# Kotstantinovskiy/SonicDiffusionBayesLab

Hardware: AMD Instinct MI355X
Metric: 512x512 images/sec at 50 DDIM steps (higher is better)
Workload: dtype bf16; 1 GPU; SD-1.5 512x512 DDIM 50 steps, CFG 7.5, batch=8/GPU (BASELINE configs[1]); global_batch=8, sample_size=64, parallelism=batch-shard x1, weights=SD-1.5-shaped synthetic seed 1234

## Files before the change

include/sd_hip.h:

```cpp
#ifndef SD_HIP_H
#define SD_HIP_H

#ifdef __cplusplus
extern "C" {
#endif

typedef struct sd_unet sd_unet;

typedef struct sd_unet_config {
    int sample_size;
    int in_channels;
    int out_channels;
    int num_levels;
    int block_out_channels[8];
    int layers_per_block;
    int attn_levels[8];
    int cross_attention_dim;
    int num_heads;
    int norm_num_groups;
    float norm_eps;
    int context_len;
    int weight_dtype;
    float fp8_act_scale_norm;
    float fp8_act_scale_ff;
// ... 123 lines not shown
                   int Cin, int Cout);
int sd_op_time_embedding(void* stream, float t, const void* W1, const float* b1, const void* W2, const float* b2,
                         float* scratch, float* temb, int dim_in, int dim);
int sd_op_timestep_cond(void* stream, float t, const float* cond, const void* Wc, float* row, float* emb, int cond_dim,
                        int dim);

int sd_op_ln_partials(int kind, int M, int N);
int sd_op_gemm_rowstats(void* stream, const void* X, long long ldx, const void* W, const float* bias, const void* R,
                        long long ldr, void* C, long long ldc, int M, int N, int K, float* rowstats);
int sd_op_gemm_ln(void* stream, const void* X, long long ldx, const void* Wg, const float* c1, const float* c2,
                  const float* rowstats, int parts, float eps, void* C, long long ldc, int M, int N, int K, int epi);
int sd_op_gemm_plan(void* stream, const void* X, long long ldx, const void* X2, long long ldx2, int K1, const void* W,
                    const float* bias, const float* bias2, const void* R, long long ldr, void* C, long long ldc, int M, int N,
                    int K, float* rowstats, float* stats, const float* ln_rs, int ln_parts, const float* ln_c1, float ln_eps,
                    void* KV, int hm_tokens);
int sd_op_xattn_fused_rowstats(void* stream, const void* X, const void* R, void* Y, const void* At, const void* Bw,
                               const float* bias, int M, int C, int rows_per_sample, int L, float* rowstats);
int sd_op_xattn_fused(void* stream, const void* X, const void* R, void* Y, const void* At, const void* Bw,
                      const float* bias, int M, int C, int rows_per_sample, int L);
int sd_op_xattn_fused_ln(void* stream, const void* X, const void* R, void* Y, const void* At, const void* Bw,
                         const float* bias, int M, int C, int rows_per_sample, int L, const float* ln_rowstats, int ln_parts,
                         long long ln_rows, const float* c2, float eps, float* rowstats);
int sd_op_conv3x3_ablate(void* stream, const void* X, const void* W, void* Y, int B, int Hin, int Win, int Cin, int Cout,
                         int ablate);
int sd_op_xattn_fused_stamps(void* stream, const void* X, const void* R, void* Y, const void* At, const void* Bw,
                             const float* bias, int M, int C, int rows_per_sample, int L, unsigned long long* stamps);

int sd_op_gemm_fp8(void* stream, const void* X, long long ldx, const void* W, const float* wscale, float xscale,
                   const float* bias, const void* R, long long ldr, void* C, long long ldc, int M, int N, int K, int epi,
                   int out_fp8, float oscale);
// ... 14 lines not shown
```

sonicdiffusionbayeslab_amd/_lib.py:

```python
from __future__ import annotations

import ctypes as C
import os
import re
from typing import Optional

HERE = os.path.dirname(os.path.abspath(__file__))
LIB_PATH = os.environ.get("SD_AMD_LIB", os.path.join(HERE, "lib", "libsdhip.so"))
HEADER_PATH = os.path.normpath(os.path.join(HERE, "..", "include", "sd_hip.h"))

ABLATE_LIB_PATH = os.path.join(HERE, "lib", "libsdhip_ablate.so")

_lib: Optional[C.CDLL] = None
_ablate: Optional[C.CDLL] = None


class SdUnetConfig(C.Structure):
    _fields_ = [
        ("sample_size", C.c_int), ("in_channels", C.c_int), ("out_channels", C.c_int),
        ("num_levels", C.c_int), ("block_out_channels", C.c_int * 8), ("layers_per_block", C.c_int),
        ("attn_levels", C.c_int * 8), ("cross_attention_dim", C.c_int), ("num_heads", C.c_int),
        ("norm_num_groups", C.c_int), ("norm_eps", C.c_float), ("context_len", C.c_int),
        ("weight_dtype", C.c_int), ("fp8_act_scale_norm", C.c_float), ("fp8_act_scale_ff", C.c_float),
        ("time_cond_proj_dim", C.c_int),
# ... 68 lines not shown
    "sd_op_conv3x3_kernel": (_i, [_i, _i, _i, _i, _i, _i, _i, _i]),
    "sd_op_softmax_rows": (_i, [_vp, _vp, _ll, _i, _f]),
    "sd_op_layernorm": (_i, [_vp, _vp, _vp, _vp, _vp, _i, _i, _f]),
    "sd_op_attention": (_i, [_vp, _vp, _ll, _vp, _ll, _vp, _ll, _vp, _ll, _i, _i, _i, _i, _i, _f]),
    "sd_op_gemm_qkv_headmajor": (_i, [_vp, _vp, _ll, _vp, _vp, _vp, _i, _i, _i, _i]),
    "sd_op_attention_headmajor": (_i, [_vp, _vp, _ll, _vp, _vp, _vp, _ll, _i, _i, _i, _i, _i, _f]),
    "sd_op_clip_attention": (_i, [_vp, _vp, _vp, _i, _i, _i, _i]),
    "sd_op_conv_in": (_i, [_vp, _vp, _i, _vp, _vp, _vp, _i, _i, _i, _i, _i]),
    "sd_op_conv_out": (_i, [_vp, _vp, _vp, _vp, _vp, _i, _i, _i, _i, _i]),
    "sd_op_time_embedding": (_i, [_vp, _f, _vp, _vp, _vp, _vp, _vp, _vp, _i, _i]),
    "sd_op_timestep_cond": (_i, [_vp, _f, _vp, _vp, _vp, _vp, _i, _i]),
    "sd_op_ln_partials": (_i, [_i, _i, _i]),
    "sd_op_gemm_rowstats": (_i, [_vp, _vp, _ll, _vp, _vp, _vp, _ll, _vp, _ll, _i, _i, _i, _vp]),
    "sd_op_gemm_plan": (_i, [_vp, _vp, _ll, _vp, _ll, _i, _vp, _vp, _vp, _vp, _ll, _vp, _ll, _i, _i, _i, _vp, _vp, _vp, _i, _vp, _f,
                            _vp, _i]),
    "sd_op_gemm_ln": (_i, [_vp, _vp, _ll, _vp, _vp, _vp, _vp, _i, _f, _vp, _ll, _i, _i, _i, _i]),
    "sd_op_xattn_fused_rowstats": (_i, [_vp, _vp, _vp, _vp, _vp, _vp, _vp, _i, _i, _i, _i, _vp]),
    "sd_op_xattn_fused": (_i, [_vp, _vp, _vp, _vp, _vp, _vp, _vp, _i, _i, _i, _i]),
    "sd_op_xattn_fused_ln": (_i, [_vp, _vp, _vp, _vp, _vp, _vp, _vp, _i, _i, _i, _i, _vp, _i, _ll, _vp, _f, _vp]),
    "sd_op_xattn_fused_stamps": (_i, [_vp, _vp, _vp, _vp, _vp, _vp, _vp, _i, _i, _i, _i, _vp]),
    "sd_op_gemm_fp8": (_i, [_vp, _vp, _ll, _vp, _vp, _f, _vp, _vp, _ll, _vp, _ll, _i, _i, _i, _i, _i, _f]),
    "sd_op_conv3x3_fp8": (_i, [_vp, _vp, _vp, _vp, _f, _vp, _vp, _vp, _vp, _i, _i, _i, _i, _i, _i, _i]),
    "sd_op_groupnorm_fp8": (_i, [_vp, _vp, _i, _vp, _i, _vp, _vp, _vp, _i, _i, _i, _f, _i, _i, _f]),
    "sd_op_layernorm_fp8": (_i, [_vp, _vp, _vp, _vp, _vp, _i, _i, _i, _f, _f]),
    "sd_op_quantize_fp8": (_i, [_vp, _vp, _vp, _ll, _i, _i, _f]),
}


def load() -> C.CDLL:
    global _lib
# ... 44 lines not shown
```

sonicdiffusionbayeslab_amd/csrc/gemm_conv.hip:

```cpp
#include "common.h"
#include "kernels.h"

#include <stdlib.h>

#ifdef SD_ABLATE
#define SD_TUNE(p) ((p).tune)
#else
#define SD_TUNE(p) 0
#endif

namespace {

constexpr int AMODE_GEMM = 0;
constexpr int AMODE_CONV = 1;
constexpr int EPI_STD = 0;
constexpr int EPI_GEGLU = 1;
constexpr int EPI_SOFTMAX = 2;

constexpr int kPersistentGrid = 512;

template <int N>
__device__ __forceinline__ void wait_vmcnt() {
    asm volatile("s_waitcnt vmcnt(%0)" ::"n"(N) : "memory");
}
// ... 629 lines not shown

int sd_gemm_splitk(int M, int N, int K, int rows) {
    static const char* env = getenv("SD_SPLITK");
    if (env) return atoi(env) > 1 ? atoi(env) : 1;
    if (rows == 0) rows = sd_gemm_tile_rows(M, N, K);
    const int tiles = ((M + rows - 1) / rows) * ((N + 159) / 160);
    const int KT = K / 64;
    if (tiles >= 448) return 1;
    int want = (512 + tiles - 1) / tiles;
    int maxs = KT / 12;
    int s = want < maxs ? want : maxs;
    if (s > 8) s = 8;
    return s < 1 ? 1 : s;
}

static int check_fp8(const GemmArgs& a, const char* what) {
    SD_REQUIRE(a.wscale != nullptr && a.xscale_inv > 0.f, "%s fp8: weight scales / activation scale missing", what);
    SD_REQUIRE(a.K % 128 == 0 && a.K >= 128, "%s fp8: K=%d must be a positive multiple of 128", what, a.K);
    SD_REQUIRE(a.X2 == nullptr && a.K1 == a.K, "%s fp8: no second K segment", what);
    SD_REQUIRE(a.rows_per_batch == 0, "%s fp8: per-sample weights are bf16 only", what);
    SD_REQUIRE(((uintptr_t)a.X & 15) == 0 && ((uintptr_t)a.W & 15) == 0, "%s fp8: operands must be 16-byte aligned", what);
    return 0;
}

static int check_stats(const GemmArgs& a, int epi) {
    if (!a.stats) return 0;
    SD_REQUIRE(epi == EPI_STD && a.M % 64 == 0 && !(a.splitk > 1 && a.slab) && !a.out_fp8,
               "producer statistics: plain epilogue, M %% 64 == 0 and no split-K (M=%d splitk=%d)", a.M, a.splitk);
    return 0;
}
// ... 41 lines not shown
        SD_REQUIRE(a.N % 32 == 0, "geglu gemm: N=%d must be a multiple of 32", a.N);
        if (!lean_off && big_tile_mode() == 0 && sd_gemm_lean_applicable(a, 1)) return sd_launch_gemm_lean(a, 1, 256, stream);
        if (big_tile_ok(a.M, a.N, 128)) return launch<256, 128, 4, 2, 3, AMODE_GEMM, EPI_GEGLU>(a, stream);
        if (big_tile_mode() != 3 && a.N % 256 == 0) return launch<256, 256, 4, 2, 2, AMODE_GEMM, EPI_GEGLU>(a, stream);
        return launch<128, 128, 2, 2, 2, AMODE_GEMM, EPI_GEGLU>(a, stream);
    }
    SD_REQUIRE(a.rows_per_batch == 0 || a.rows_per_batch % 128 == 0,
               "gemm: rows_per_batch=%d must be a multiple of the 128-row tile", a.rows_per_batch);
    if (epi == EPI_SOFTMAX) {
        SD_REQUIRE(a.N % 80 == 0 && a.sm_valid > 0 && a.sm_valid <= 80 && a.R == nullptr && (a.bias == nullptr || a.ln_rs),
                   "softmax gemm: N=%d must be a multiple of 80, 0 < sm_valid=%d <= 80, no bias/residual", a.N, a.sm_valid);
        SD_REQUIRE(!a.ln_per_sample || (a.ln_rs && a.rows_per_batch > 0), "gemm: per-sample LayerNorm vectors need per-sample weights");
        return launch<128, 160, 2, 2, 2, AMODE_GEMM, EPI_SOFTMAX>(a, stream);
    }
    if (a.rows_per_batch) return launch<128, 160, 2, 2, 2, AMODE_GEMM, EPI_STD>(a, stream);
    if (!lean_off && big_tile_mode() == 0 && sd_gemm_lean_applicable(a, epi)) {
        const int rows = (!a.stats && !a.ln_rs && !a.hm_C) ? sd_gemm_tile_rows(a.M, a.N, a.K) : 128;
        return sd_launch_gemm_lean(a, 0, rows, stream);
    }
    if (big_tile_ok(a.M, a.N, 160)) return launch<256, 160, 4, 2, 3, AMODE_GEMM, EPI_STD>(a, stream);
    if (big_tile_mode() == 2) return launch<256, 160, 4, 2, 2, AMODE_GEMM, EPI_STD>(a, stream);
    if (!a.stats && !a.ln_rs && sd_gemm_tile_rows(a.M, a.N, a.K) == 64) return launch<64, 160, 2, 2, 2, AMODE_GEMM, EPI_STD>(a, stream);
    return launch<128, 160, 2, 2, 2, AMODE_GEMM, EPI_STD>(a, stream);
}

int sd_launch_conv3x3(const GemmArgs& a, hipStream_t stream) {
    if (check_stats(a, EPI_STD)) return -1;
    if (a.dt == 1) {
        if (check_fp8(a, "conv3x3")) return -1;
        SD_REQUIRE(a.Cin % 128 == 0, "conv3x3 fp8: Cin=%d must be a multiple of 128 (pad the channels)", a.Cin);
// ... 30 lines not shown
```

sonicdiffusionbayeslab_amd/csrc/gemm_lean.hip:

```cpp
#include "common.h"
#include "kernels.h"
#include <mutex>
#include <stdlib.h>

namespace {

typedef __amdgpu_buffer_rsrc_t rsrc_t;

struct LeanArgs {
    const void* X; const void* X2; const void* W; const void* R; void* C; void* KV;
    const float* vec0; const float* vec1;
    const float* ln_rs; float* rowstats; float* stats;
    unsigned x_bytes, x2_bytes, w_bytes, r_bytes, c_bytes, kv_bytes;
    int M, N, K, K1;
    int ldxb, ldx2b, ldwb, ldrb, ldcb;
    int tiles_m, tiles_n;
    float ln_eps, inv_k;
    int hm_tpc;
    int hm_tok_shift, hm_heads, hm_samples;
};

template <int N>
__device__ __forceinline__ void wait_vmcnt() {
    asm volatile("s_waitcnt vmcnt(%0)" ::"n"(N) : "memory");
}

__device__ __forceinline__ rsrc_t make_rsrc(const void* p, unsigned bytes) {
    return __builtin_amdgcn_make_buffer_rsrc((void*)p, 0, (int)bytes, 0x00020000);
}
__device__ __forceinline__ void dma16(rsrc_t r, void* lds_wave_base, int voff, int soff) {
    __builtin_amdgcn_raw_ptr_buffer_load_lds(r, LDS_PTR(lds_wave_base), 16, voff, soff, 0, 0);
}

template <int BM, int BN, int WAVES_M, int WAVES_N, int NP, bool GEGLU>
__global__ __launch_bounds__(WAVES_M* WAVES_N * 64, 2) void gemm_lean_kernel(const LeanArgs p) {
    constexpr bool LN = NP > 0;
    constexpr int NW = WAVES_M * WAVES_N;
    constexpr int WTM = BM / WAVES_M, WTN = BN / WAVES_N;
    constexpr int TM = WTM / 16, TN = WTN / 16;
    constexpr int XI = BM / 8, WI = BN / 8;
    static_assert(XI % NW == 0 && WI % NW == 0, "pieces split evenly over the waves");
    constexpr int XPW = XI / NW, WPW = WI / NW;
    constexpr int STAGE_BYTES = (BM + BN) * 128;
    static_assert(GEGLU ? TN % 4 == 0 : TN % 2 == 1, "store schedule: GEGLU pairs of output tiles; std TN / 2 paired + one 8-byte store");
    constexpr bool FRAG_DB = TM * TN * 4 + (TM + TN) * 8 <= 200;
    constexpr int TNH = GEGLU ? TN / 2 : TN;

    extern __shared__ __attribute__((aligned(16))) char smem[];
    char* lnbuf = smem + 2 * STAGE_BYTES;
    char* vecs = lnbuf + NW * 512;

    const int tid = threadIdx.x, lane = tid & 63;
    const int wave = __builtin_amdgcn_readfirstlane(tid >> 6);
    const int wm = wave % WAVES_M, wn = wave / WAVES_M;
    const int lrow = lane & 15, lq = lane >> 4;

    const int nblk = gridDim.x;
    int work;
    {
        const int q = nblk >> 3, r = nblk & 7, xcd = blockIdx.x & 7, idx = blockIdx.x >> 3;
        work = (xcd < r ? xcd * (q + 1) : r * (q + 1) + (xcd - r) * q) + idx;
    }
    const int nwork = p.tiles_m * p.tiles_n;
    if (work >= nwork) return;
// ... 18 lines not shown
        const int hl = (cl * 205) >> 13;
        vH[j] = ((hl << p.hm_tok_shift) + rowl) * 80 + (cl - hl * 40) * 2;
    }
    const int vLn = (wm * WTM + lane) * 8;
    const int vRs = rowl * 8;
    const int vSt = (wn * WTN + lq * 4) * 8;
    const int vVec = (wn * WTN + lane * 4) * 4;

    const int swz[2] = {((lq) ^ (lane & 7)) << 4, ((4 + lq) ^ (lane & 7)) << 4};
    const int xoff = (wm * WTM + lrow) * 128;
    const int woff = BM * 128 + (wn * WTN + lrow) * 128;

    const int KT = p.K >> 6;
    int m0 = tile_m * BM, n0 = tile_n * BN;

    auto stage = [&](int kt, int buf) {
        char* xs = smem + buf * STAGE_BYTES;
        char* ws = xs + BM * 128;
        const int k0 = kt * 64;
        if (LN || k0 < p.K1) {
            const int so = (m0 + wave * 8) * p.ldxb + k0 * 2;
#pragma unroll
            for (int i = 0; i < XPW; ++i) dma16(rX, xs + (wave + i * NW) * 1024, vX, so + i * (NW * 8) * p.ldxb);
        } else {
            const int so = (m0 + wave * 8) * p.ldx2b + (k0 - p.K1) * 2;
#pragma unroll
            for (int i = 0; i < XPW; ++i) dma16(rX2, xs + (wave + i * NW) * 1024, vX2, so + i * (NW * 8) * p.ldx2b);
        }
        const int sw = (n0 + wave * 8) * p.ldwb + k0 * 2;
#pragma unroll
// ... 7 lines not shown
        for (int t = 0; t < TM; ++t) xf[t] = *(const bf16x8*)(sb + xoff + t * 2048 + swz[ks]);
#pragma unroll
        for (int t = 0; t < TN; ++t) wf[t] = *(const bf16x8*)(sb + woff + t * 2048 + swz[ks]);
    };
    auto mfmas = [&](const bf16x8* xf, const bf16x8* wf) {
#pragma unroll
        for (int a = 0; a < TN; ++a)
#pragma unroll
            for (int b = 0; b < TM; ++b)
                acc[a][b] = __builtin_amdgcn_mfma_f32_16x16x32_bf16(wf[a], xf[b], acc[a][b], 0, 0, 0);
    };

    constexpr int EPI_STORES = GEGLU ? (TN / 4) * TM : (TN / 2 + 1) * TM;
    int g = 0;
    bool stores_pending = false;
    stage(0, 0);
    while (true) {
#pragma unroll
        for (int a = 0; a < TN; ++a)
#pragma unroll
            for (int b = 0; b < TM; ++b) acc[a][b] = f32x4{0.f, 0.f, 0.f, 0.f};
        for (int kt = 0; kt < KT - 1; ++kt) {
            if (kt == 0 && stores_pending) wait_vmcnt<EPI_STORES>();
            else wait_vmcnt<0>();
            __builtin_amdgcn_s_barrier();
            asm volatile("" ::: "memory");
            const char* sb = smem + ((g + kt) & 1) * STAGE_BYTES;
            load_frags(sb, 0, xf0, wf0);
            __builtin_amdgcn_sched_barrier(0);
            stage(kt + 1, (g + kt + 1) & 1);
            if (kt == 0 && wm == 0 && lane < WTN / 4) {
                glds16((const char*)p.vec0 + (long)n0 * 4 + (unsigned)vVec, vecs + wn * WTN * 4);
                glds16((const char*)p.vec1 + (long)n0 * 4 + (unsigned)vVec, vecs + BN * 4 + wn * WTN * 4);
            }
            __builtin_amdgcn_sched_barrier(0);
            if (FRAG_DB) {
                load_frags(sb, 1, xf1, wf1);
                mfmas(xf0, wf0);
                mfmas(xf1, wf1);
            } else {
                mfmas(xf0, wf0);
                load_frags(sb, 1, xf0, wf0);
                mfmas(xf0, wf0);
            }
        }
        wait_vmcnt<0>();
        __builtin_amdgcn_s_barrier();
        asm volatile("" ::: "memory");
        static_assert(!LN || WTM == 64, "LayerNorm fold: lane l owns row l of its wave's 64 rows");
        u32x2 ep[LN ? NP : (GEGLU ? 1 : TN * TM)];
        {
            const char* sb = smem + ((g + KT - 1) & 1) * STAGE_BYTES;
            load_frags(sb, 0, xf0, wf0);
            if (FRAG_DB) load_frags(sb, 1, xf1, wf1);
            if (LN) {
                const char* src = (const char*)p.ln_rs + (long)m0 * 8;
#pragma unroll
                for (int i = 0; i < NP; ++i) ep[i] = *(const u32x2*)((src + (long)i * p.M * 8) + (unsigned)vLn);
            } else if (!GEGLU && p.R) {
                const int so = m0 * p.ldrb + n0 * 2;
#pragma unroll
                for (int b = 0; b < TM; ++b)
#pragma unroll
                    for (int a = 0; a < TN; ++a)
                        ep[a * TM + b] = __builtin_bit_cast(u32x2, __builtin_amdgcn_raw_buffer_load_b64(rR, vR + a * 32, so + b * 16 * p.ldrb, 0));
            }
            __builtin_amdgcn_sched_barrier(0);
// ... 55 lines not shown
                for (int a = 0; a < TNH; ++a) {
                    const f32x4 bv = v0[a] + v1[a];
#pragma unroll
                    for (int b = 0; b < TM; ++b) acc[a0 + a][b] += bv;
                }
            }
        }

        const int em0 = m0, en0 = n0, etile_n = tile_n;
        work += nblk;
        const bool more = work < nwork;
        if (more) {
            tile_n += dn; tile_m += dm;
            if (tile_n >= p.tiles_n) { tile_n -= p.tiles_n; tile_m += 1; }
            m0 = tile_m * BM; n0 = tile_n * BN;
            stage(0, g & 1);
            stores_pending = true;
        }

        if (!LN && !GEGLU && WTM == 64 && p.stats) {
            char* dst = (char*)p.stats + ((long)((em0 + wm * WTM) >> 6) * p.N + en0) * 8 + (unsigned)vSt;
#pragma unroll
            for (int a = 0; a < TN; ++a) {
                float sv[4] = {0.f, 0.f, 0.f, 0.f}, qv[4] = {0.f, 0.f, 0.f, 0.f};
#pragma unroll
                for (int b = 0; b < TM; ++b) {
                    const unsigned p0 = pack2bf(acc[a][b][0], acc[a][b][1]), p1 = pack2bf(acc[a][b][2], acc[a][b][3]);
                    const float v[4] = {bflo(p0), bfhi(p0), bflo(p1), bfhi(p1)};
#pragma unroll
                    for (int j = 0; j < 4; ++j) { sv[j] += v[j]; qv[j] = __builtin_fmaf(v[j], v[j], qv[j]); }
                }
// ... 93 lines not shown
    if (hipGetDevice(&dev) != hipSuccess || dev < 0 || dev >= 16) return nullptr;
    std::lock_guard<std::mutex> lock(mu);
    if (!z[dev]) {
        float* p = nullptr;
        float probe = 1.f;
        if (hipMalloc((void**)&p, 16384 * 4) != hipSuccess) return nullptr;
        if (hipMemset(p, 0, 16384 * 4) != hipSuccess || hipMemcpy(&probe, p + 16383, 4, hipMemcpyDeviceToHost) != hipSuccess || probe != 0.f) {
            (void)hipFree(p);
            return nullptr;
        }
        z[dev] = p;
    }
    return z[dev];
}

template <int BM, int BN, int WAVES_M, int WAVES_N, int NP, bool GEGLU>
int launch_lean(const LeanArgs& a0, hipStream_t stream) {
    LeanArgs a = a0;
    a.tiles_m = (a.M + BM - 1) / BM;
    a.tiles_n = a.N / BN;
    constexpr int NW = WAVES_M * WAVES_N;
    constexpr int smem = 2 * (BM + BN) * 128 + NW * 512 + 2 * BN * 4;
    static_assert(smem <= 160 * 1024, "tile does not fit the 160 KiB LDS");
    auto kern = gemm_lean_kernel<BM, BN, WAVES_M, WAVES_N, NP, GEGLU>;
    static bool attr_set = false;
    if (!attr_set) {
        SD_CHECK_HIP(hipFuncSetAttribute((const void*)kern, hipFuncAttributeMaxDynamicSharedMemorySize, smem));
        attr_set = true;
    }
    int grid = a.tiles_m * a.tiles_n;
    constexpr int resident = smem > 80 * 1024 ? 256 : 512;
    if (grid > resident) grid = resident;
    hipLaunchKernelGGL(kern, dim3(grid), dim3(NW * 64), smem, stream, a);
    SD_CHECK_HIP(hipGetLastError());
    return 0;
}

}

// ... 10 lines not shown
    if (a.R && (long)a.M * a.ldr * 2 >= big) return false;
    if ((a.stats || a.rowstats || a.ln_rs || a.hm_C) && a.M % (epi ? 256 : 128) != 0) return false;
    if (a.ln_rs) {
        if (a.R || a.bias2 || !a.bias || !a.ln_c1 || a.X2 || a.K1 != a.K || a.stats || a.rowstats) return false;
        if (a.ln_np != 2 && a.ln_np != 4 && a.ln_np != 8 && a.ln_np != 16) return false;
    }
    if (epi == 1 && (a.R || a.bias2 || a.X2 || a.K1 != a.K || a.stats || a.rowstats || a.hm_C)) return false;
    if (a.hm_C) {
        if (!a.ln_rs || !a.KV || a.hm_C % 160 != 0 || a.N != 3 * a.hm_C || a.hm_tok < 128 || (a.hm_tok & (a.hm_tok - 1)) ||
            a.M % a.hm_tok != 0 || (long)a.M * a.hm_C * 4 >= big)
            return false;
    }
    return true;
}

int sd_launch_gemm_lean(const GemmArgs& g, int epi, int rows, hipStream_t stream) {
    SD_REQUIRE(sd_gemm_lean_applicable(g, epi), "gemm (lean): problem not supported (M=%d N=%d K=%d epi=%d)", g.M, g.N, g.K, epi);
    SD_REQUIRE(epi == 1 || rows == 128 || (rows == 64 && !g.stats && !g.ln_rs && !g.hm_C),
               "gemm (lean): %d-row tile with block statistics / LayerNorm fold / head-major K|V", rows);
    const long ldw = g.ldw ? g.ldw : g.K;
    LeanArgs a{};
    a.X = g.X; a.X2 = g.X2; a.W = g.W; a.R = g.R; a.C = g.C; a.KV = g.KV;
    a.M = g.M; a.N = g.N; a.K = g.K; a.K1 = g.K1;
    a.ldxb = (int)g.ldx * 2; a.ldx2b = (int)g.ldx2 * 2; a.ldwb = (int)ldw * 2; a.ldrb = (int)g.ldr * 2; a.ldcb = (int)g.ldc * 2;
    a.x_bytes = (unsigned)(((long)g.M - 1) * g.ldx * 2 + (long)g.K1 * 2);
    a.x2_bytes = g.X2 ? (unsigned)(((long)g.M - 1) * g.ldx2 * 2 + (long)(g.K - g.K1) * 2) : 0;
    a.w_bytes = (unsigned)(((long)g.N - 1) * ldw * 2 + (long)g.K * 2);
    a.r_bytes = g.R ? (unsigned)(((long)g.M - 1) * g.ldr * 2 + (long)g.N * 2) : 0;
    const int ncols = epi ? g.N / 2 : g.hm_C ? g.hm_C : g.N;
    a.c_bytes = (unsigned)(((long)g.M - 1) * g.ldc * 2 + (long)ncols * 2);
    a.kv_bytes = g.hm_C ? (unsigned)((long)g.M * g.hm_C * 4) : 0;
    const float* zeros = nullptr;
    if (!g.bias || (!g.ln_rs && !g.bias2)) {
        zeros = zero_vector();
// ... 5 lines not shown
        a.vec0 = g.bias ? g.bias : zeros; a.vec1 = g.bias2 ? g.bias2 : zeros;
    }
    a.rowstats = g.rowstats; a.stats = g.stats;
    if (g.hm_C) {
        a.hm_tpc = g.hm_C / 160;
        int sh = 0;
        while ((1 << sh) < g.hm_tok) ++sh;
        a.hm_tok_shift = sh; a.hm_heads = g.hm_C / 40; a.hm_samples = g.M / g.hm_tok;
    }
    if (epi == 1) {
        if (!g.ln_rs) return launch_lean<256, 256, 4, 2, 0, true>(a, stream);
        return g.ln_np == 2 ? launch_lean<256, 256, 4, 2, 2, true>(a, stream)
             : g.ln_np == 4 ? launch_lean<256, 256, 4, 2, 4, true>(a, stream)
             : g.ln_np == 8 ? launch_lean<256, 256, 4, 2, 8, true>(a, stream) : launch_lean<256, 256, 4, 2, 16, true>(a, stream);
    }
    if (g.ln_rs)
        return g.ln_np == 2 ? launch_lean<128, 160, 2, 2, 2, false>(a, stream)
             : g.ln_np == 4 ? launch_lean<128, 160, 2, 2, 4, false>(a, stream)
             : g.ln_np == 8 ? launch_lean<128, 160, 2, 2, 8, false>(a, stream) : launch_lean<128, 160, 2, 2, 16, false>(a, stream);
    return rows == 64 ? launch_lean<64, 160, 2, 2, 0, false>(a, stream) : launch_lean<128, 160, 2, 2, 0, false>(a, stream);
}
```

sonicdiffusionbayeslab_amd/csrc/kernels.h:

```cpp
#pragma once
#include "common.h"

struct GemmArgs {
    const bf16_t* X = nullptr;
    long ldx = 0;
    const bf16_t* X2 = nullptr;
    long ldx2 = 0;
    int K1 = 0;
    const bf16_t* W = nullptr;
    long ldw = 0;
    const float* bias = nullptr;
    const float* bias2 = nullptr;
    const bf16_t* R = nullptr;
    long ldr = 0;
    bf16_t* C = nullptr;
    long ldc = 0;
    int M = 0, N = 0, K = 0;
    int Hin = 0, Win = 0, Cin = 0, Hout = 0, Wout = 0, stride = 1, up = 0;
    int splitk = 1;
    float* slab = nullptr;
    int defer_reduce = 0;
    const void* zero_page = nullptr;
    long w_batch_stride = 0;
    int rows_per_batch = 0;
// ... 3 lines not shown
    float* stats = nullptr;
    float* rowstats = nullptr;
    bf16_t* KV = nullptr;
    int hm_C = 0, hm_tok = 0;
    int subpix = 0;
    const float* ln_rs = nullptr;
    const float* ln_c1 = nullptr;
    int ln_np = 0;
    float ln_eps = 1e-5f;
    int ln_per_sample = 0;
    int dt = 0;
    const float* wscale = nullptr;
    float xscale_inv = 1.0f;
    int out_fp8 = 0;
    float oscale = 1.0f;
};

int sd_gemm_tile_rows(int M, int N, int K = 0);
int sd_gemm_splitk(int M, int N, int K, int rows = 0);
int sd_launch_gemm(const GemmArgs& a, int epi , hipStream_t stream);
int sd_launch_conv3x3(const GemmArgs& a, hipStream_t stream);
bool sd_gemm_lean_applicable(const GemmArgs& a, int epi);
int sd_launch_gemm_lean(const GemmArgs& a, int epi, int rows, hipStream_t stream);
void sd_launch_splitk_reduce(const GemmArgs& a, hipStream_t stream);
bool sd_conv_halo_applicable(const GemmArgs& a);
int sd_conv_halo_mode(const GemmArgs& a);
int sd_conv3x3_splitk(int M, int N, int Cin, int Hin, int Win, int stride, int up, int dt = 0);
bool sd_conv_halo_subpix_applicable(const GemmArgs& a);
int sd_launch_conv3x3_halo(const GemmArgs& a, hipStream_t stream);

struct GroupNormArgs {
    const bf16_t* x1 = nullptr; int C1 = 0;
    const bf16_t* x2 = nullptr; int C2 = 0;
    const float* gamma = nullptr; const float* beta = nullptr;
    bf16_t* y = nullptr;
    int out_fp8 = 0, Cpad = 0;
    float oscale = 1.0f;
    const float* stats1 = nullptr; const float* stats2 = nullptr;
// ... 96 lines not shown
```

sonicdiffusionbayeslab_amd/csrc/unet.hip:

```cpp
#include "../../include/sd_hip.h"
#include "common.h"
#include "kernels.h"

#include <stdarg.h>
#include <stdio.h>
#include <stdlib.h>
#include <string.h>
#include <sys/mman.h>

#include <algorithm>
#include <chrono>
#include <map>
#include <new>
#include <string>
#include <thread>
#include <tuple>
#include <unordered_map>
#include <vector>

static thread_local char g_err[1024] = "";
void sd_set_error(const char* fmt, ...) {
    va_list ap;
    va_start(ap, fmt);
    vsnprintf(g_err, sizeof(g_err), fmt, ap);
// ... 63 lines not shown
    long ldq = 0, ldk = 0, ldv = 0, ldo = 0, qoff = 0, koff = 0, voff = 0;
    int silu_in = 0, splitk = 1;
    int defer = 0, slab_t = -1, slab_k = 0, slab_r = -1, slab_b2t = -1;
    size_t slab_b = NOFF;
    long slab_b2idx = 0;
    int wt = -1;
    size_t wx = NOFF;
    long xoff = 0, woff_el = 0, coff = 0, ldx_o = 0, ldw_o = 0, ldc_o = 0;
    float scale = 0.f;
    long wbs = 0;
    int rpb = 0, sm_valid = 0;
    int dt = 0, out_fp8 = 0, Cpad = 0, Kalg = 0;
    int sname = -1;
    int stats = -1, s1 = -1, s2 = -1;
    int subpix = 0;
    int hm = 0;
    int qps = 0;
    int rs = -1, lnrs = -1, lnnp = 0;
    size_t c1 = NOFF;
    size_t wsc = NOFF;
    float xs = 1.f, os = 1.f;
    int nwrap = 0;
    Wrap wraps[3];
};

struct HostBlob {
    unsigned char* p = nullptr;
    size_t n = 0, cap = 0;
    unsigned char* data() { return p; }
    const unsigned char* data() const { return p; }
// ... 767 lines not shown
        return it->second;
    }
    bool producer_stats = !(getenv("SD_GN_PRODUCER_STATS") && atoi(getenv("SD_GN_PRODUCER_STATS")) == 0);
    void want_stats(Op& o, int M, int N) {
        if (!producer_stats || u->kind != 0 || o.splitk > 1 || M % 64 != 0 || o.epi != 0 || o.rpb != 0) return;
        o.stats = tensor((size_t)(M / 64) * N * 2 * 4);
        stats_of[o.out] = o.stats;
    }

    int prefix_rep = 1;
    int replicate(int t, size_t bytes, int r) {
        Op o; o.kind = OP_REPLICATE; o.x1 = t; o.M = (int)(bytes / 16); o.N = r; o.out = tensor(bytes * r);
        push(o);
        return o.out;
    }
    bool ln_fold = !(getenv("SD_LN_FOLD") && atoi(getenv("SD_LN_FOLD")) == 0);
    int want_rowstats(Op& o, int M, int C, int& rs) {
        int np = 0;
        if (o.kind == OP_GEMM && o.epi == 0 && o.splitk == 1 && !o.out_fp8 && o.N == C && o.M == M && o.ldc_o == 0) np = (C + 159) / 160 * 2;
        else if (o.kind == OP_XATTN && o.N == C && o.M == M) np = 2 * sd_xattn_slices(M, C);
        static const bool big_tiles = getenv("SD_GEMM_BIG") != nullptr;
        if (!ln_fold || np == 0 || np > 16 || C < 128 || big_tiles) return 0;
        o.rs = rs = tensor((size_t)np * M * 2 * 4);
        return np;
    }
    int gemm_ln(int x, int rs, int np, int M, int N, int C, const std::string& w, int epi) {
        Op o; o.kind = OP_GEMM; o.x1 = x; o.K1 = o.K = o.Kalg = C; o.M = M; o.N = N; o.epi = epi; o.splitk = 1;
        o.w = W(w + ".ln"); o.c1 = W(w + ".c1"); o.b = W(w + ".c2"); o.lnrs = rs; o.lnnp = np;
        o.out = tensor((size_t)M * (epi ? N / 2 : N) * 2);
        push(o);
        return o.out;
    }

    int ctx_tensor(size_t bytes) {
        const int id = tensor(bytes, true);
        pl.tensors[id].ctx = true;
        return id;
    }
    int tensor(size_t bytes, bool persistent = false) {
        Tn t;
        t.bytes = (bytes + 255) / 256 * 256;
        t.persistent = persistent;
        pl.tensors.push_back(t);
// ... 56 lines not shown
        if (o.splitk > 1) o.aux = tensor((size_t)o.splitk * o.M * o.N * 4);
        o.out = tensor((size_t)o.M * cout * 2);
        GemmArgs g;
        g.M = o.M; g.N = o.N; g.Cin = o.Cin; g.K = o.K; g.ldw = o.K; g.Hin = hin; g.Win = win; g.Hout = o.Hout; g.Wout = o.Wout;
        g.stride = stride; g.up = up; g.dt = o.dt;
        if (sd_conv_halo_mode(g) != 2) want_stats(o, o.M, cout);
        push(o);
        return o.out;
    }
    int gemm(int x1, int k1, int x2, int k2, int M, int N, const std::string& w, const std::string& b, int r, int epi,
             bool fq = false, const std::string& oname = "") {
        Op o; o.kind = OP_GEMM; o.x1 = x1; o.x2 = x2; o.K1 = k1; o.K = k1 + k2; o.Kalg = o.K; o.M = M; o.N = N; o.epi = epi;
        o.b = b.empty() ? NOFF : W(b); o.r = r;
        if (fq) { o.dt = 1; o.K = o.K1 = pad128(k1); o.w = W(w + ".fp8"); o.wsc = W(w + ".scale"); o.xs = xscale(x1); }
        else o.w = W(w);
        o.splitk = epi ? 1 : sd_gemm_splitk(M, N, o.dt ? o.K / 2 : o.K, o.dt ? 128 : 0);
        if (o.splitk > 1) o.aux = tensor((size_t)o.splitk * M * N * 4);
        if (!oname.empty()) {
            o.out_fp8 = 1; o.sname = u->act_id(oname, u->s_ff); o.os = u->act_scale[o.sname]; o.Cpad = pad128(N / 2);
            o.out = tensor((size_t)M * o.Cpad); tscale[o.out] = o.os;
        } else o.out = tensor((size_t)M * (epi ? N / 2 : N) * 2);
        push(o);
        return o.out;
    }
    int ln(int x, int M, int C, const std::string& g, const std::string& b, bool fq = false) {
        Op o; o.kind = OP_LN; o.x1 = x; o.M = M; o.N = C; o.g = W(g); o.be = W(b); o.eps = 1e-5f;
        if (fq) {
            o.out_fp8 = 1; o.Cpad = pad128(C); o.sname = u->act_id(stem(g), u->s_norm); o.os = u->act_scale[o.sname];
            o.out = tensor((size_t)M * o.Cpad); tscale[o.out] = o.os;
        } else o.out = tensor((size_t)M * C * 2);
        push(o);
// ... 109 lines not shown
        int ff;
        if (!fq && (np = want_rowstats(pl.ops.back(), M, C, rs)) > 0) {
            ff = gemm_ln(h2, rs, np, M, 8 * C, C, t + "ff.geglu.weight", 1);
        } else {
            int n3 = ln(h2, M, C, t + "norm3.weight", t + "norm3.bias", fq);
            ff = gemm(n3, C, -1, 0, M, 8 * C, t + "ff.geglu.weight", t + "ff.geglu.bias", -1, 1, fq, fq ? t + "ff.net.0" : std::string());
        }
        static const bool merge_off = getenv("SD_FF_MERGE") && atoi(getenv("SD_FF_MERGE")) == 0;
        int out;
        if (!fq && !merge_off) {
            out = gemm(ff, 4 * C, h2, C, M, C, p + "ff_out.weight", p + "ff_out.bias", x, 0);
        } else {
            int h3 = gemm(ff, 4 * C, -1, 0, M, C, t + "ff.net.2.weight", t + "ff.net.2.bias", h2, 0, fq);
            out = gemm(h3, C, -1, 0, M, C, p + "proj_out.weight", p + "proj_out.bias", x, 0);
        }
        if (pl.ops.back().splitk == 1 && sd_gemm_tile_rows(M, C, pl.ops.back().K) == 128) want_stats(pl.ops.back(), M, C);
        return out;
    }

    int vae_resnet(const std::string& p, int x, int cin, int cout, int rh, int rw) {
        const int hw = rh * rw, M = UB * hw;
        int t1 = gn(x, cin, -1, 0, hw, p + "norm1.weight", p + "norm1.bias", 1e-6f, 1);
        int t2 = conv3(t1, rh, rw, cin, cout, 1, 0, p + "conv1.weight", p + "conv1.bias", 0, -1, -1);
        int t3 = gn(t2, cout, -1, 0, hw, p + "norm2.weight", p + "norm2.bias", 1e-6f, 1);
        int sc = x;
        if (cin != cout) sc = gemm(x, cin, -1, 0, M, cout, p + "conv_shortcut.weight", p + "conv_shortcut.bias", -1, 0);
        return conv3(t3, rh, rw, cout, cout, 1, 0, p + "conv2.weight", p + "conv2.bias", 0, -1, sc);
    }
    int vae_attention(const std::string& p, int x, int C, int rh, int rw) {
        const int hw = rh * rw, M = UB * hw;
        const int qc = hw <= 4096 ? hw : 2048;
// ... 386 lines not shown
            a.ldx = o.ldx_o ? o.ldx_o : o.K1; a.X2 = (const bf16_t*)T(o.x2); a.ldx2 = o.K - o.K1; a.K1 = o.K1;
            a.W = o.wt >= 0 ? (const bf16_t*)T(o.wt) + o.woff_el : (const bf16_t*)(wb + o.w); a.ldw = o.ldw_o;
            a.bias = o.b != NOFF ? (const float*)(wb + o.b) : nullptr;
            a.R = (const bf16_t*)T(o.r); a.ldr = o.N; a.C = (bf16_t*)T(o.out) + o.coff;
            a.ldc = o.ldc_o ? o.ldc_o : (o.epi == 1 ? o.N / 2 : o.N);
            a.M = o.M; a.N = o.N; a.K = o.K; a.zero_page = g_zero_page; a.splitk = o.splitk; a.slab = (float*)T(o.aux);
            a.defer_reduce = o.defer;
            a.w_batch_stride = o.wbs; a.rows_per_batch = o.rpb; a.sm_valid = o.sm_valid;
            if (o.dt) { a.dt = 1; a.wscale = (const float*)(wb + o.wsc); a.xscale_inv = 1.0f / o.xs; }
            if (o.out_fp8) { a.out_fp8 = 1; a.oscale = o.os; a.ldc = o.Cpad; }
            a.stats = (float*)T(o.stats);
            a.rowstats = (float*)T(o.rs);
            if (o.hm) { a.hm_C = o.N / 3; a.hm_tok = o.HW; a.ldc = a.hm_C; a.KV = (bf16_t*)T(o.out) + (long)o.M * a.hm_C; }
            if (o.lnrs >= 0) { a.ln_rs = (const float*)T(o.lnrs); a.ln_np = o.lnnp; a.ln_c1 = (const float*)(wb + o.c1); a.ln_eps = 1e-5f; }
            if (o.lnrs >= 0 && o.s1 >= 0) { a.ln_c1 = (const float*)T(o.s1); a.bias = (const float*)T(o.s2); a.ln_per_sample = 1; }
            return sd_launch_gemm(a, o.epi, stream);
        }
        case OP_LN:
            if (o.out_fp8)
                return sd_launch_layernorm_fp8((const bf16_t*)T(o.x1), (const float*)(wb + o.g), (const float*)(wb + o.be),
                                               T(o.out), o.M, o.N, o.Cpad, o.eps, o.os, stream);
            return sd_launch_layernorm((const bf16_t*)T(o.x1), (const float*)(wb + o.g), (const float*)(wb + o.be),
                                       (bf16_t*)T(o.out), o.M, o.N, o.eps, stream);
        case OP_ATTN: {
            AttnArgs a;
            a.Q = (const bf16_t*)T(o.x1) + o.qoff; a.ldq = o.ldq;
            a.K = (const bf16_t*)T(o.x2) + o.koff; a.ldk = o.ldk;
            a.V = (const bf16_t*)T(o.x2) + o.voff; a.ldv = o.ldv;
            a.O = (bf16_t*)T(o.out); a.ldo = o.ldo;
            a.B = o.B; a.heads = o.heads; a.Nq = o.Nq; a.Nk = o.Nk; a.D = o.D;
// ... 945 lines not shown

extern "C" int sd_op_ln_partials(int kind, int M, int N) { return kind == 0 ? (N + 159) / 160 * 2 : 2 * sd_xattn_slices(M, N); }
extern "C" int sd_op_gemm_rowstats(void* stream, const void* X, long long ldx, const void* W, const float* bias, const void* R,
                                   long long ldr, void* C, long long ldc, int M, int N, int K, float* rowstats) {
    if (ensure_zero_page()) return -2;
    SD_REQUIRE(rowstats, "sd_op_gemm_rowstats: null partials buffer");
    GemmArgs a;
    a.X = (const bf16_t*)X; a.ldx = ldx; a.K1 = K; a.W = (const bf16_t*)W; a.bias = bias; a.R = (const bf16_t*)R; a.ldr = ldr;
    a.C = (bf16_t*)C; a.ldc = ldc; a.M = M; a.N = N; a.K = K; a.zero_page = g_zero_page; a.splitk = 1; a.rowstats = rowstats;
    return sd_launch_gemm(a, 0, (hipStream_t)stream);
}
extern "C" int sd_op_gemm_plan(void* stream, const void* X, long long ldx, const void* X2, long long ldx2, int K1, const void* W,
                               const float* bias, const float* bias2, const void* R, long long ldr, void* C, long long ldc,
                               int M, int N, int K, float* rowstats, float* stats, const float* ln_rs, int ln_parts,
                               const float* ln_c1, float ln_eps, void* KV, int hm_tokens) {
    if (ensure_zero_page()) return -2;
    GemmArgs a;
    a.X = (const bf16_t*)X; a.ldx = ldx; a.X2 = (const bf16_t*)X2; a.ldx2 = ldx2; a.K1 = K1; a.W = (const bf16_t*)W;
    a.bias = bias; a.bias2 = bias2; a.R = (const bf16_t*)R; a.ldr = ldr; a.C = (bf16_t*)C; a.ldc = ldc; a.M = M; a.N = N; a.K = K;
    a.zero_page = g_zero_page; a.splitk = 1; a.rowstats = rowstats; a.stats = stats;
    a.ln_rs = ln_rs; a.ln_np = ln_parts; a.ln_c1 = ln_c1; a.ln_eps = ln_eps;
    if (hm_tokens > 0) {
        SD_REQUIRE(N % 3 == 0 && KV, "sd_op_gemm_plan: head-major K / V needs N = 3 C and a KV buffer");
        a.KV = (bf16_t*)KV; a.hm_C = N / 3; a.hm_tok = hm_tokens;
    }
    return sd_launch_gemm(a, 0, (hipStream_t)stream);
}
extern "C" int sd_op_gemm_ln(void* stream, const void* X, long long ldx, const void* Wg, const float* c1, const float* c2,
                             const float* rowstats, int parts, float eps, void* C, long long ldc, int M, int N, int K, int epi) {
    if (ensure_zero_page()) return -2;
    SD_REQUIRE(epi == 0 || epi == 1, "sd_op_gemm_ln: epi %d (0 = plain, 1 = GEGLU)", epi);
    GemmArgs a;
    a.X = (const bf16_t*)X; a.ldx = ldx; a.K1 = K; a.W = (const bf16_t*)Wg; a.bias = c2;
    a.C = (bf16_t*)C; a.ldc = ldc; a.M = M; a.N = N; a.K = K; a.zero_page = g_zero_page; a.splitk = 1;
    a.ln_rs = rowstats; a.ln_np = parts; a.ln_c1 = c1; a.ln_eps = eps;
    return sd_launch_gemm(a, epi, (hipStream_t)stream);
}

extern "C" int sd_op_xattn_fused_rowstats(void* stream, const void* X, const void* R, void* Y, const void* At, const void* Bw,
// ... 40 lines not shown
```

Baseline: 11.19 images/s.

## Add a 4-stage LDS ring variant of the lean GEMM for small-M wide GEMMs

Adds a STAGES template parameter to the lean GEMM kernel so the standard 128x160 tile can prefetch up to three K-tiles ahead, using counted vmcnt waits instead of waiting for all loads. The planner routes std-epilogue bf16 GEMMs with M<=4096 and enough tiles to this deep ring, and disables split-K and block stats on those ops. The aim is to hide global-load latency on GEMMs with few tiles per CU. In exchange it doubles LDS per block and drops to one block per CU in launch bounds, which can cut occupancy.

```diff
diff --git a/include/sd_hip.h b/include/sd_hip.h
--- a/include/sd_hip.h
+++ b/include/sd_hip.h
@@ -161,6 +161,10 @@
                     const float* bias, const float* bias2, const void* R, long long ldr, void* C, long long ldc, int M, int N,
                     int K, float* rowstats, float* stats, const float* ln_rs, int ln_parts, const float* ln_c1, float ln_eps,
                     void* KV, int hm_tokens);
+int sd_op_gemm_plan_deep(void* stream, const void* X, long long ldx, const void* X2, long long ldx2, int K1, const void* W,
+                         const float* bias, const float* bias2, const void* R, long long ldr, void* C, long long ldc, int M,
+                         int N, int K, float* rowstats, float* stats, const float* ln_rs, int ln_parts, const float* ln_c1,
+                         float ln_eps, void* KV, int hm_tokens, int deep);
 int sd_op_xattn_fused_rowstats(void* stream, const void* X, const void* R, void* Y, const void* At, const void* Bw,
                                const float* bias, int M, int C, int rows_per_sample, int L, float* rowstats);
 int sd_op_xattn_fused(void* stream, const void* X, const void* R, void* Y, const void* At, const void* Bw,
diff --git a/sonicdiffusionbayeslab_amd/_lib.py b/sonicdiffusionbayeslab_amd/_lib.py
--- a/sonicdiffusionbayeslab_amd/_lib.py
+++ b/sonicdiffusionbayeslab_amd/_lib.py
@@ -106,6 +106,8 @@
     "sd_op_gemm_rowstats": (_i, [_vp, _vp, _ll, _vp, _vp, _vp, _ll, _vp, _ll, _i, _i, _i, _vp]),
     "sd_op_gemm_plan": (_i, [_vp, _vp, _ll, _vp, _ll, _i, _vp, _vp, _vp, _vp, _ll, _vp, _ll, _i, _i, _i, _vp, _vp, _vp, _i, _vp, _f,
                             _vp, _i]),
+    "sd_op_gemm_plan_deep": (_i, [_vp, _vp, _ll, _vp, _ll, _i, _vp, _vp, _vp, _vp, _ll, _vp, _ll, _i, _i, _i, _vp, _vp, _vp, _i, _vp,
+                                 _f, _vp, _i, _i]),
     "sd_op_gemm_ln": (_i, [_vp, _vp, _ll, _vp, _vp, _vp, _vp, _i, _f, _vp, _ll, _i, _i, _i, _i]),
     "sd_op_xattn_fused_rowstats": (_i, [_vp, _vp, _vp, _vp, _vp, _vp, _vp, _i, _i, _i, _i, _vp]),
     "sd_op_xattn_fused": (_i, [_vp, _vp, _vp, _vp, _vp, _vp, _vp, _i, _i, _i, _i]),
diff --git a/sonicdiffusionbayeslab_amd/csrc/gemm_conv.hip b/sonicdiffusionbayeslab_amd/csrc/gemm_conv.hip
--- a/sonicdiffusionbayeslab_amd/csrc/gemm_conv.hip
+++ b/sonicdiffusionbayeslab_amd/csrc/gemm_conv.hip
@@ -667,6 +667,11 @@
     return s < 1 ? 1 : s;
 }
 
+bool sd_gemm_deep_route(int M, int N, int K) {
+    if (M > 4096 || N % 160 != 0 || K < 128) return false;
+    return ((M + 127) / 128) * (N / 160) >= 192;
+}
+
 static int check_fp8(const GemmArgs& a, const char* what) {
     SD_REQUIRE(a.wscale != nullptr && a.xscale_inv > 0.f, "%s fp8: weight scales / activation scale missing", what);
     SD_REQUIRE(a.K % 128 == 0 && a.K >= 128, "%s fp8: K=%d must be a positive multiple of 128", what, a.K);
@@ -738,6 +743,8 @@
         return launch<128, 160, 2, 2, 2, AMODE_GEMM, EPI_SOFTMAX>(a, stream);
     }
     if (a.rows_per_batch) return launch<128, 160, 2, 2, 2, AMODE_GEMM, EPI_STD>(a, stream);
+    if (!lean_off && big_tile_mode() == 0 && a.deep && epi == EPI_STD && sd_gemm_deep_applicable(a))
+        return sd_launch_gemm_lean(a, 0, 128, stream, true);
     if (!lean_off && big_tile_mode() == 0 && sd_gemm_lean_applicable(a, epi)) {
         const int rows = (!a.stats && !a.ln_rs && !a.hm_C) ? sd_gemm_tile_rows(a.M, a.N, a.K) : 128;
         return sd_launch_gemm_lean(a, 0, rows, stream);
diff --git a/sonicdiffusionbayeslab_amd/csrc/gemm_lean.hip b/sonicdiffusionbayeslab_amd/csrc/gemm_lean.hip
--- a/sonicdiffusionbayeslab_amd/csrc/gemm_lean.hip
+++ b/sonicdiffusionbayeslab_amd/csrc/gemm_lean.hip
@@ -32,8 +32,8 @@
     __builtin_amdgcn_raw_ptr_buffer_load_lds(r, LDS_PTR(lds_wave_base), 16, voff, soff, 0, 0);
 }
 
-template <int BM, int BN, int WAVES_M, int WAVES_N, int NP, bool GEGLU>
-__global__ __launch_bounds__(WAVES_M* WAVES_N * 64, 2) void gemm_lean_kernel(const LeanArgs p) {
+template <int BM, int BN, int WAVES_M, int WAVES_N, int NP, bool GEGLU, int STAGES = 2>
+__global__ __launch_bounds__(WAVES_M* WAVES_N * 64, STAGES > 2 ? 1 : 2) void gemm_lean_kernel(const LeanArgs p) {
     constexpr bool LN = NP > 0;
     constexpr int NW = WAVES_M * WAVES_N;
     constexpr int WTM = BM / WAVES_M, WTN = BN / WAVES_N;
@@ -42,12 +42,14 @@
     static_assert(XI % NW == 0 && WI % NW == 0, "pieces split evenly over the waves");
     constexpr int XPW = XI / NW, WPW = WI / NW;
     constexpr int STAGE_BYTES = (BM + BN) * 128;
+    static_assert(STAGES >= 2 && STAGES <= 4 && (STAGES == 2 || !GEGLU), "ring depth: 2, or 3 / 4 for the std tile");
+    constexpr int PER_TILE = XPW + WPW;
     static_assert(GEGLU ? TN % 4 == 0 : TN % 2 == 1, "store schedule: GEGLU pairs of output tiles; std TN / 2 paired + one 8-byte store");
     constexpr bool FRAG_DB = TM * TN * 4 + (TM + TN) * 8 <= 200;
     constexpr int TNH = GEGLU ? TN / 2 : TN;
 
     extern __shared__ __attribute__((aligned(16))) char smem[];
-    char* lnbuf = smem + 2 * STAGE_BYTES;
+    char* lnbuf = smem + STAGES * STAGE_BYTES;
     char* vecs = lnbuf + NW * 512;
 
     const int tid = threadIdx.x, lane = tid & 63;
@@ -96,6 +98,7 @@
     const int KT = p.K >> 6;
     int m0 = tile_m * BM, n0 = tile_n * BN;
 
+    auto slot = [](int t) { return STAGES == 2 ? (t & 1) : t % STAGES; };
     auto stage = [&](int kt, int buf) {
         char* xs = smem + buf * STAGE_BYTES;
         char* ws = xs + BM * 128;
@@ -133,21 +136,41 @@
     constexpr int EPI_STORES = GEGLU ? (TN / 4) * TM : (TN / 2 + 1) * TM;
     int g = 0;
     bool stores_pending = false;
-    stage(0, 0);
+    constexpr int LEAD = STAGES - 1;
+    auto stage_first = [&]() {
+#pragma unroll
+        for (int s = 0; s < LEAD; ++s)
+            if (s < KT) stage(s, slot(g + s));
+    };
+    auto wait_tile = [&](int kt, bool with_stores) {
+        const int ahead = KT - 1 - kt < STAGES - 2 ? KT - 1 - kt : STAGES - 2;
+        if (with_stores) {
+            if (ahead >= 2) wait_vmcnt<2 * PER_TILE + EPI_STORES>();
+            else if (ahead == 1) wait_vmcnt<PER_TILE + EPI_STORES>();
+            else wait_vmcnt<EPI_STORES>();
+        } else {
+            if (ahead >= 2) wait_vmcnt<2 * PER_TILE>();
+            else if (ahead == 1) wait_vmcnt<PER_TILE>();
+            else wait_vmcnt<0>();
+        }
+    };
+    static_assert(STAGES <= 4 && 2 * PER_TILE + EPI_STORES <= 63, "counted waits: vmcnt is 6 bits");
+    stage_first();
     while (true) {
 #pragma unroll
         for (int a = 0; a < TN; ++a)
 #pragma unroll
             for (int b = 0; b < TM; ++b) acc[a][b] = f32x4{0.f, 0.f, 0.f, 0.f};
         for (int kt = 0; kt < KT - 1; ++kt) {
-            if (kt == 0 && stores_pending) wait_vmcnt<EPI_STORES>();
+            if (STAGES > 2) wait_tile(kt, kt == 0 && stores_pending);
+            else if (kt == 0 && stores_pending) wait_vmcnt<EPI_STORES>();
             else wait_vmcnt<0>();
             __builtin_amdgcn_s_barrier();
             asm volatile("" ::: "memory");
-            const char* sb = smem + ((g + kt) & 1) * STAGE_BYTES;
+            const char* sb = smem + slot(g + kt) * STAGE_BYTES;
             load_frags(sb, 0, xf0, wf0);
             __builtin_amdgcn_sched_barrier(0);
-            stage(kt + 1, (g + kt + 1) & 1);
+            if (kt + LEAD < KT) stage(kt + LEAD, slot(g + kt + LEAD));
             if (kt == 0 && wm == 0 && lane < WTN / 4) {
                 glds16((const char*)p.vec0 + (long)n0 * 4 + (unsigned)vVec, vecs + wn * WTN * 4);
                 glds16((const char*)p.vec1 + (long)n0 * 4 + (unsigned)vVec, vecs + BN * 4 + wn * WTN * 4);
@@ -169,7 +192,7 @@
         static_assert(!LN || WTM == 64, "LayerNorm fold: lane l owns row l of its wave's 64 rows");
         u32x2 ep[LN ? NP : (GEGLU ? 1 : TN * TM)];
         {
-            const char* sb = smem + ((g + KT - 1) & 1) * STAGE_BYTES;
+            const char* sb = smem + slot(g + KT - 1) * STAGE_BYTES;
             load_frags(sb, 0, xf0, wf0);
             if (FRAG_DB) load_frags(sb, 1, xf1, wf1);
             if (LN) {
@@ -255,7 +278,7 @@
             tile_n += dn; tile_m += dm;
             if (tile_n >= p.tiles_n) { tile_n -= p.tiles_n; tile_m += 1; }
             m0 = tile_m * BM; n0 = tile_n * BN;
-            stage(0, g & 1);
+            stage_first();
             stores_pending = true;
         }
 
@@ -379,15 +402,15 @@
     return z[dev];
 }
 
-template <int BM, int BN, int WAVES_M, int WAVES_N, int NP, bool GEGLU>
+template <int BM, int BN, int WAVES_M, int WAVES_N, int NP, bool GEGLU, int STAGES = 2>
 int launch_lean(const LeanArgs& a0, hipStream_t stream) {
     LeanArgs a = a0;
     a.tiles_m = (a.M + BM - 1) / BM;
     a.tiles_n = a.N / BN;
     constexpr int NW = WAVES_M * WAVES_N;
-    constexpr int smem = 2 * (BM + BN) * 128 + NW * 512 + 2 * BN * 4;
+    constexpr int smem = STAGES * (BM + BN) * 128 + NW * 512 + 2 * BN * 4;
     static_assert(smem <= 160 * 1024, "tile does not fit the 160 KiB LDS");
-    auto kern = gemm_lean_kernel<BM, BN, WAVES_M, WAVES_N, NP, GEGLU>;
+    auto kern = gemm_lean_kernel<BM, BN, WAVES_M, WAVES_N, NP, GEGLU, STAGES>;
     static bool attr_set = false;
     if (!attr_set) {
         SD_CHECK_HIP(hipFuncSetAttribute((const void*)kern, hipFuncAttributeMaxDynamicSharedMemorySize, smem));
@@ -428,10 +451,16 @@
     return true;
 }
 
-int sd_launch_gemm_lean(const GemmArgs& g, int epi, int rows, hipStream_t stream) {
+bool sd_gemm_deep_applicable(const GemmArgs& a) {
+    return sd_gemm_lean_applicable(a, 0) && (!a.ln_rs || a.ln_np == 16);
+}
+
+int sd_launch_gemm_lean(const GemmArgs& g, int epi, int rows, hipStream_t stream, bool deep) {
     SD_REQUIRE(sd_gemm_lean_applicable(g, epi), "gemm (lean): problem not supported (M=%d N=%d K=%d epi=%d)", g.M, g.N, g.K, epi);
     SD_REQUIRE(epi == 1 || rows == 128 || (rows == 64 && !g.stats && !g.ln_rs && !g.hm_C),
                "gemm (lean): %d-row tile with block statistics / LayerNorm fold / head-major K|V", rows);
+    SD_REQUIRE(!deep || (sd_gemm_deep_applicable(g) && epi == 0 && rows == 128),
+               "gemm (lean, deep ring): std epilogue on 128-row tiles, LayerNorm fold with 16 partials only (np=%d)", g.ln_np);
     const long ldw = g.ldw ? g.ldw : g.K;
     LeanArgs a{};
     a.X = g.X; a.X2 = g.X2; a.W = g.W; a.R = g.R; a.C = g.C; a.KV = g.KV;
@@ -467,6 +496,8 @@
              : g.ln_np == 4 ? launch_lean<256, 256, 4, 2, 4, true>(a, stream)
              : g.ln_np == 8 ? launch_lean<256, 256, 4, 2, 8, true>(a, stream) : launch_lean<256, 256, 4, 2, 16, true>(a, stream);
     }
+    if (deep)
+        return g.ln_rs ? launch_lean<128, 160, 2, 2, 16, false, 4>(a, stream) : launch_lean<128, 160, 2, 2, 0, false, 4>(a, stream);
     if (g.ln_rs)
         return g.ln_np == 2 ? launch_lean<128, 160, 2, 2, 2, false>(a, stream)
              : g.ln_np == 4 ? launch_lean<128, 160, 2, 2, 4, false>(a, stream)
diff --git a/sonicdiffusionbayeslab_amd/csrc/kernels.h b/sonicdiffusionbayeslab_amd/csrc/kernels.h
--- a/sonicdiffusionbayeslab_amd/csrc/kernels.h
+++ b/sonicdiffusionbayeslab_amd/csrc/kernels.h
@@ -41,6 +41,7 @@
     float xscale_inv = 1.0f;
     int out_fp8 = 0;
     float oscale = 1.0f;
+    int deep = 0;
 };
 
 int sd_gemm_tile_rows(int M, int N, int K = 0);
@@ -48,7 +49,9 @@
 int sd_launch_gemm(const GemmArgs& a, int epi , hipStream_t stream);
 int sd_launch_conv3x3(const GemmArgs& a, hipStream_t stream);
 bool sd_gemm_lean_applicable(const GemmArgs& a, int epi);
-int sd_launch_gemm_lean(const GemmArgs& a, int epi, int rows, hipStream_t stream);
+bool sd_gemm_deep_applicable(const GemmArgs& a);
+int sd_launch_gemm_lean(const GemmArgs& a, int epi, int rows, hipStream_t stream, bool deep = false);
+bool sd_gemm_deep_route(int M, int N, int K);
 void sd_launch_splitk_reduce(const GemmArgs& a, hipStream_t stream);
 bool sd_conv_halo_applicable(const GemmArgs& a);
 int sd_conv_halo_mode(const GemmArgs& a);
diff --git a/sonicdiffusionbayeslab_amd/csrc/unet.hip b/sonicdiffusionbayeslab_amd/csrc/unet.hip
--- a/sonicdiffusionbayeslab_amd/csrc/unet.hip
+++ b/sonicdiffusionbayeslab_amd/csrc/unet.hip
@@ -101,6 +101,7 @@
     int sname = -1;
     int stats = -1, s1 = -1, s2 = -1;
     int subpix = 0;
+    int deep = 0;
     int hm = 0;
     int qps = 0;
     int rs = -1, lnrs = -1, lnnp = 0;
@@ -898,6 +899,7 @@
         push(o);
         return o.out;
     }
+    bool deep_on = !(getenv("SD_GEMM_DEEP") && atoi(getenv("SD_GEMM_DEEP")) == 0);
     bool ln_fold = !(getenv("SD_LN_FOLD") && atoi(getenv("SD_LN_FOLD")) == 0);
     int want_rowstats(Op& o, int M, int C, int& rs) {
         int np = 0;
@@ -911,6 +913,7 @@
     int gemm_ln(int x, int rs, int np, int M, int N, int C, const std::string& w, int epi) {
         Op o; o.kind = OP_GEMM; o.x1 = x; o.K1 = o.K = o.Kalg = C; o.M = M; o.N = N; o.epi = epi; o.splitk = 1;
         o.w = W(w + ".ln"); o.c1 = W(w + ".c1"); o.b = W(w + ".c2"); o.lnrs = rs; o.lnnp = np;
+        o.deep = deep_on && epi == 0 && np == 16 && sd_gemm_deep_route(M, N, C);
         o.out = tensor((size_t)M * (epi ? N / 2 : N) * 2);
         push(o);
         return o.out;
@@ -997,7 +1000,8 @@
         o.b = b.empty() ? NOFF : W(b); o.r = r;
         if (fq) { o.dt = 1; o.K = o.K1 = pad128(k1); o.w = W(w + ".fp8"); o.wsc = W(w + ".scale"); o.xs = xscale(x1); }
         else o.w = W(w);
-        o.splitk = epi ? 1 : sd_gemm_splitk(M, N, o.dt ? o.K / 2 : o.K, o.dt ? 128 : 0);
+        o.deep = deep_on && !fq && epi == 0 && sd_gemm_deep_route(M, N, o.K);
+        o.splitk = epi || o.deep ? 1 : sd_gemm_splitk(M, N, o.dt ? o.K / 2 : o.K, o.dt ? 128 : 0);
         if (o.splitk > 1) o.aux = tensor((size_t)o.splitk * M * N * 4);
         if (!oname.empty()) {
             o.out_fp8 = 1; o.sname = u->act_id(oname, u->s_ff); o.os = u->act_scale[o.sname]; o.Cpad = pad128(N / 2);
@@ -1137,7 +1141,7 @@
             int h3 = gemm(ff, 4 * C, -1, 0, M, C, t + "ff.net.2.weight", t + "ff.net.2.bias", h2, 0, fq);
             out = gemm(h3, C, -1, 0, M, C, p + "proj_out.weight", p + "proj_out.bias", x, 0);
         }
-        if (pl.ops.back().splitk == 1 && sd_gemm_tile_rows(M, C, pl.ops.back().K) == 128) want_stats(pl.ops.back(), M, C);
+        if (pl.ops.back().splitk == 1 && !pl.ops.back().deep && sd_gemm_tile_rows(M, C, pl.ops.back().K) == 128) want_stats(pl.ops.back(), M, C);
         return out;
     }
 
@@ -1554,6 +1558,7 @@
             if (o.hm) { a.hm_C = o.N / 3; a.hm_tok = o.HW; a.ldc = a.hm_C; a.KV = (bf16_t*)T(o.out) + (long)o.M * a.hm_C; }
             if (o.lnrs >= 0) { a.ln_rs = (const float*)T(o.lnrs); a.ln_np = o.lnnp; a.ln_c1 = (const float*)(wb + o.c1); a.ln_eps = 1e-5f; }
             if (o.lnrs >= 0 && o.s1 >= 0) { a.ln_c1 = (const float*)T(o.s1); a.bias = (const float*)T(o.s2); a.ln_per_sample = 1; }
+            a.deep = o.deep;
             return sd_launch_gemm(a, o.epi, stream);
         }
         case OP_LN:
@@ -2529,6 +2534,13 @@
                                const float* bias, const float* bias2, const void* R, long long ldr, void* C, long long ldc,
                                int M, int N, int K, float* rowstats, float* stats, const float* ln_rs, int ln_parts,
                                const float* ln_c1, float ln_eps, void* KV, int hm_tokens) {
+    return sd_op_gemm_plan_deep(stream, X, ldx, X2, ldx2, K1, W, bias, bias2, R, ldr, C, ldc, M, N, K, rowstats, stats, ln_rs,
+                                ln_parts, ln_c1, ln_eps, KV, hm_tokens, 0);
+}
+extern "C" int sd_op_gemm_plan_deep(void* stream, const void* X, long long ldx, const void* X2, long long ldx2, int K1,
+                                    const void* W, const float* bias, const float* bias2, const void* R, long long ldr, void* C,
+                                    long long ldc, int M, int N, int K, float* rowstats, float* stats, const float* ln_rs,
+                                    int ln_parts, const float* ln_c1, float ln_eps, void* KV, int hm_tokens, int deep) {
     if (ensure_zero_page()) return -2;
     GemmArgs a;
     a.X = (const bf16_t*)X; a.ldx = ldx; a.X2 = (const bf16_t*)X2; a.ldx2 = ldx2; a.K1 = K1; a.W = (const bf16_t*)W;
@@ -2538,6 +2550,10 @@
     if (hm_tokens > 0) {
         SD_REQUIRE(N % 3 == 0 && KV, "sd_op_gemm_plan: head-major K / V needs N = 3 C and a KV buffer");
         a.KV = (bf16_t*)KV; a.hm_C = N / 3; a.hm_tok = hm_tokens;
+    }
+    if (deep) {
+        a.deep = 1;
+        SD_REQUIRE(sd_gemm_deep_applicable(a), "sd_op_gemm_plan_deep: the deep-ring kernel does not take this problem (M=%d N=%d K=%d)", M, N, K);
     }
     return sd_launch_gemm(a, 0, (hipStream_t)stream);
 }
```

Result: no change. 11.22 images/s (median of 6 runs) (+0.2%).
